# alejandrofontan/AnyFeature-VSLAM

Measured on AMD Instinct MI355X. Metric: keypoints extracted+matched /sec (ORB32, 640x480), higher is better.
Workload: dtype u8; 1 GPU; ORB32 640x480 synthetic corners frames (LCG), 1000 kp/frame budget, 8 levels x1.2, FAST 20; extract+describe on device, brute-force Hamming match frame t vs t-1 (TH 75, ratio 0.6, orientation check); parallelism=frames sharded x1

## Files before the change

### anyfeature-vslam_amd/_lib.py

```python
import ctypes as C
import os

import numpy as np

_HERE = os.path.dirname(os.path.abspath(__file__))
LIB_PATH = os.path.join(_HERE, "libafv_hip.so")


def use_library(path):
    global LIB_PATH
    if _lib is not None:
        raise RuntimeError("the library is already loaded")
    LIB_PATH = os.path.abspath(path)


ABI_VERSION = 6
MAX_LEVELS = 8
DESC_BYTES = 32
OK, EINVAL, ENODEV, ENOMEM, EHIP, ECAPACITY, EUNSUPPORTED, ETIMEOUT = 0, -1, -2, -3, -4, -5, -6, -7
MATCH_KF_KF, MATCH_KF_FRAME = 0, 1
MATCH_FLOAT32 = 0x100
PROJ_LOCALMAP, PROJ_LASTFRAME = 0, 1
STAGES = ("pyramid", "fast_nms", "select_quadtree", "describe", "match_topk", "match_resolve", "retain_harris")

# ... 228 lines not shown
    "afv_points_set_descriptors": (_i, [_vp, _vp, _i, _vp]),
    "afv_points_set_descriptors_from_table": (_i, [_vp, _vp, _i, _vp, _vp, _vp]),
    "afv_points_get": (_i, [_vp, _vp, _i, _vp, _vp, _vp, _vp, _vp, _vp, _vp, _vp, _vp]),
    "afv_frame_set_pose": (_i, [_vp, _vp, _vp, _vp, _f, _f, _f, _f, _f]),
    "afv_frame_search_points": (_i, [_vp, C.POINTER(PointSearch), _vp, _vp, _vp, C.POINTER(C.c_int32)]),
    "afv_frame_fuse_points": (_i, [_vp, C.POINTER(PointSearch), _i, _vp, _vp]),
    "afv_frame_project_points": (_i, [_vp, C.POINTER(PointSearch), C.POINTER(PointProjection)]),
    "afv_frame_pose_optimize": (_i, [_vp, _vp, C.POINTER(PoseJob), _i, C.POINTER(PoseResult)]),
    "afv_table_set_scale": (_i, [_vp, _i, _vp, _vp, _vp, _vp]),
    "afv_table_triangulate": (_i, [_vp, _vp, _vp, C.POINTER(TriPointsJob), _i, _vp, _vp, C.c_int32, _vp, _vp, _vp, _vp, _vp]),
    "afv_table_create_new_points": (_i, [_vp, C.c_int32, _vp, _i, C.POINTER(TableTriJob), C.POINTER(TriPointsJob), _vp, _vp, _vp, C.c_int32,
                                         _vp, _vp, _vp, _vp, _vp, _vp, C.POINTER(C.c_int32)]),
    "afv_table_sim3_hypotheses": (_i, [_vp, _vp, _vp, _vp, C.POINTER(Sim3Job), _i, _vp, _vp, _vp, _vp, _i, _i, _vp, _vp, _vp, _vp, _vp, _vp,
                                       _vp, _vp, _vp]),
    "afv_vocab_set_weights": (_i, [_vp, _vp, _vp, _vp]),
    "afv_bow_vector": (_i, [_vp, _vp, _vp, _i, _vp, _vp, C.POINTER(C.c_int32)]),
    "afv_frame_get_bowvec": (_i, [_vp, _vp, _vp, C.POINTER(C.c_int32)]),
    "afv_table_set_bowvec": (_i, [_vp, _i, _vp, _vp, _i]),
    "afv_table_score_bow": (_i, [_vp, C.POINTER(BowQuery), _i, _vp, _vp, _vp, _vp]),
    "afv_vocab_train": (_i, [_vp, C.POINTER(VocabTrainParams), _vp, C.c_int64, _vp, _i, C.POINTER(_vp)]),
    "afv_vocab_train_device": (_i, [_vp, C.POINTER(VocabTrainParams), _vp, _sz, C.c_int64, _vp, _i, C.POINTER(_vp)]),
    "afv_vocab_tree_nnodes": (_i, [_vp]),
    "afv_vocab_tree_get": (_i, [_vp, _vp, _vp, _vp, _vp, _vp]),
    "afv_vocab_tree_stats": (_i, [_vp, _vp, _vp, _vp, C.POINTER(C.c_int32)]),
    "afv_vocab_tree_destroy": (None, [_vp]),
    "afv_hamming256": (_i, [_vp, _vp]),
    "afv_akaze_default_params": (None, [_vp]),
    "afv_akaze_create": (_i, [_i, _vp, C.POINTER(_vp)]),
    "afv_akaze_destroy": (None, [_vp]),
    "afv_akaze_last_error": (C.c_char_p, [_vp]),
    "afv_akaze_plan_for": (_i, [_vp, _i, _i, _vp]),
    "afv_akaze_scale_space": (_i, [_vp, _vp, _i, _i, _i, _i, C.c_size_t]),
    "afv_akaze_scale_space_device": (_i, [_vp, _vp, _i, _i, _i, _i, C.c_size_t]),
    "afv_akaze_synchronize": (_i, [_vp]),
    "afv_akaze_get_plane": (_i, [_vp, _i, _i, _i, _vp]),
    "afv_akaze_get_kcontrast": (_i, [_vp, _i, _vp]),
    "afv_akaze_detect": (_i, [_vp]),
    "afv_akaze_get_keypoints": (_i, [_vp, _i, _vp, _i, _vp]),
    "afv_akaze_get_candidates": (_i, [_vp, _i, _i, _vp, _i, _vp]),
    "afv_akaze_describe": (_i, [_vp]),
    "afv_akaze_get_features": (_i, [_vp, _i, _vp, _vp, _i, _vp]),
    "afv_akaze_extract": (_i, [_vp, _vp, _i, _i, _i, _i, C.c_size_t, _vp, _vp, _i, _vp]),
    "afv_akaze_extract_device": (_i, [_vp, _vp, _i, _i, _i, _i, C.c_size_t]),
    "afv_akaze_get_quotas": (_i, [_vp, _vp]),
    "afv_akaze_set_step_by_step": (_i, [_vp, _i]),
    "afv_akaze_set_suppress_engine": (_i, [_vp, _i, _i]),
    "afv_akaze_debug_neighbour_cap": (_i, [_vp, _i]),
    "afv_akaze_profile_enable": (_i, [_vp, _i]),
    "afv_akaze_profile_read": (_i, [_vp, _vp, _vp, _vp]),
    "afv_profile_enable": (_i, [_vp, _i]),
    "afv_profile_read": (_i, [_vp, _vp, _vp, _vp]),
    "afv_set_split_threshold": (_i, [_vp, _i]),
    "afv_set_split_chunks": (_i, [_vp, _i]),
    "afv_set_match_engine": (_i, [_vp, _i]),
    "afv_set_small_batch_path": (_i, [_vp, _i, _i]),
    "afv_set_match_resolve": (_i, [_vp, _i]),
    "afv_set_l2_chunk_pairs": (_i, [_vp, _i]),
    "afv_debug_pyramid_plan": (_i, [C.POINTER(OrbParams), _i, _i, _i, _i, _vp, _i, _vp, _vp, _i]),
    "afv_debug_fast_tiles": (_i, [C.POINTER(OrbParams), _i, _i, _vp, _i, _vp, C.POINTER(_i)]),
    "afv_debug_describe_reach": (_i, [_vp, _vp, _vp, _vp, _vp]),
    "afv_set_pipeline_chunk": (_i, [_vp, _i, _i]),
    "afv_get_geometry": (_i, [_vp, C.POINTER(Geometry)]),
    "afv_debug_get_level": (_i, [_vp, _i, _i, _vp]),
    "afv_debug_get_candidates": (_i, [_vp, _i, _i, _vp, _vp, _i, C.POINTER(_i)]),
    "afv_debug_get_selected": (_i, [_vp, _i, _i, _vp, _vp, _vp, _i, C.POINTER(_i)]),
    "afv_debug_blur_level": (_i, [_vp, _i, _i, _vp]),
    "afv_num_stages": (_i, []),
}

_lib = None


def load():
    global _lib
    if _lib is not None:
        return _lib
    try:
        import torch
    except ImportError:
        pass
    if not os.path.exists(LIB_PATH):
        raise ImportError("%s is missing: build the HIP extension first (python __graft_entry__.py or "
                          "anyfeature-vslam_amd/build.py); there is no CPU fallback" % LIB_PATH)
    lib = C.CDLL(LIB_PATH)
    for name, (res, args) in SYMBOLS.items():
        fn = getattr(lib, name)
        fn.restype = res
        fn.argtypes = args
    if lib.afv_abi_version() != ABI_VERSION:
        raise ImportError("%s speaks ABI revision %d, this mirror %d" % (LIB_PATH, lib.afv_abi_version(), ABI_VERSION))
    if lib.afv_num_stages() > len(STAGES):
        raise ImportError("%s reports %d profile stages, this mirror knows %d" % (LIB_PATH, lib.afv_num_stages(), len(STAGES)))
    _lib = lib
    return lib


class AfvError(RuntimeError):
    def __init__(self, code, detail=""):
        self.code = code
        msg = load().afv_strerror(code).decode()
        super().__init__("afv error %d (%s)%s" % (code, msg, (": " + detail) if detail else ""))


def strerror(code):
    return load().afv_strerror(int(code)).decode()

# ... 21 lines not shown
```

### anyfeature-vslam_amd/csrc/afv_api.hip

```cpp
#include "afv_runtime.h"

static const char *k_errors[] = {"ok", "invalid argument", "no usable HIP device", "out of memory", "HIP runtime error",
                                 "output capacity too small", "unsupported", "device-side wait timed out"};


extern "C" void afv_default_orb_params(afv_orb_params *p) {
    if (!p) return;
    p->nfeatures = 1000;
    p->nlevels = 8;
    p->scale_factor = 1.2f;
    p->fast_threshold = 20;
    p->max_width = 640;
    p->max_height = 480;
    p->max_batch = 1;
}

extern "C" int afv_abi_version(void) { return AFV_ABI_VERSION; }

extern "C" const char *afv_strerror(int code) {
    const int i = -code;
    if (i < 0 || i > 7) return "unknown error";
    return k_errors[i];
}
extern "C" const char *afv_last_error(const afv_ctx *ctx) { return ctx ? ctx->last_error.c_str() : ""; }
// ... 124 lines not shown
            float ms = 0.f;
            if (hipEventSynchronize(c->prof_ev[st][i + 1]) == hipSuccess &&
                hipEventElapsedTime(&ms, c->prof_ev[st][i], c->prof_ev[st][i + 1]) == hipSuccess) {
                c->prof_ms[st] += ms;
                c->prof_launches[st] += 1;
            }
        }
        c->prof_used[st] = 0;
    }
}

extern "C" int afv_set_split_threshold(afv_ctx *c, int min_frames) {
    if (!c || min_frames < 2) return AFV_EINVAL;
    c->split_min_frames = min_frames;
    return AFV_OK;
}
extern "C" int afv_set_pipeline_chunk(afv_ctx *c, int frames, int chunks_ahead) {
    if (!c || frames < 1 || chunks_ahead < 1 || chunks_ahead > 64) return AFV_EINVAL;
    c->pipe_chunk = frames;
    c->pipe_ahead = chunks_ahead;
    return AFV_OK;
}
extern "C" int afv_set_match_engine(afv_ctx *c, int engine) {
    if (!c || (engine != AFV_MATCH_ENGINE_POPCOUNT && engine != AFV_MATCH_ENGINE_MFMA)) return AFV_EINVAL;
    c->match_engine = engine;
    return AFV_OK;
}

extern "C" int afv_set_l2_chunk_pairs(afv_ctx *c, int pairs) {
    if (!c || pairs < 1 || pairs > 65535) return AFV_EINVAL;
    c->l2_chunk_pairs = pairs;
    return AFV_OK;
}

extern "C" int afv_set_match_resolve(afv_ctx *c, int engine) {
    if (!c || engine < 0 || engine > 2) return AFV_EINVAL;
    c->resolve_engine = engine;
    return AFV_OK;
}

extern "C" int afv_set_small_batch_path(afv_ctx *c, int mode, int max_frames) {
    if (!c || mode < 0 || mode > 2 || max_frames < 0) return AFV_EINVAL;
    c->small_mode = mode;
    if (max_frames > 0) c->small_max_frames = max_frames;
    return AFV_OK;
}

extern "C" int afv_set_split_chunks(afv_ctx *c, int chunks) {
    if (!c || (chunks != 0 && chunks < 2) || chunks > 64) return AFV_EINVAL;
    c->split_chunks = chunks;
    return AFV_OK;
}

extern "C" int afv_profile_enable(afv_ctx *c, int enable) {
    if (!c) return AFV_EINVAL;
    HIPCHK(c, hipSetDevice(c->device));
    profile_drain(c);
    c->prof = false;
    c->prof_every = enable > 0 ? enable : 0;
    c->prof_tick_extract = c->prof_tick_match = 0;
    if (enable)
        for (int st = 0; st < AFV_NUM_STAGES; ++st) {
            c->prof_ms[st] = 0.f;
            c->prof_launches[st] = 0;
            c->prof_units[st] = 0;
        }
    return AFV_OK;
}

extern "C" int afv_num_stages(void) { return AFV_NUM_STAGES; }

extern "C" int afv_profile_read(afv_ctx *c, int32_t *launches, float *total_ms, int64_t *units) {
    if (!c || !launches || !total_ms) return AFV_EINVAL;
    HIPCHK(c, hipSetDevice(c->device));
    profile_drain(c);
    for (int st = 0; st < AFV_NUM_STAGES; ++st) {
        launches[st] = c->prof_launches[st];
        total_ms[st] = c->prof_ms[st];
        if (units) units[st] = c->prof_units[st];
    }
    return AFV_OK;
}

extern "C" int afv_hamming256(const uint8_t *a, const uint8_t *b) {
    int d = 0;
    for (int i = 0; i < 8; ++i) {
        uint32_t x, y;
        std::memcpy(&x, a + 4 * i, 4);
        std::memcpy(&y, b + 4 * i, 4);
        d += __builtin_popcount(x ^ y);
    }
    return d;
}

static int validate_job(const afv_match_job &j, bool need_angles) {
    if (j.n1 < 0 || j.n2 < 0 || j.n1 > AFV_MAX_SIDE || j.n2 > AFV_MAX_SIDE) return AFV_EINVAL;
    if ((j.n1 > 0 && !j.desc1) || (j.n2 > 0 && !j.desc2)) return AFV_EINVAL;
    if (j.mode & AFV_MATCH_FLOAT32) {
        if (j.desc_bytes < 16 || j.desc_bytes > 4096 || (j.desc_bytes & 15)) return AFV_EINVAL;
    } else if (j.desc_bytes < 1 || j.desc_bytes > 64) {
        return AFV_EINVAL;
    }
    if (j.nnodes1 < 0 || j.nnodes2 < 0) return AFV_EINVAL;
    if (j.nnodes1 > 0 && (!j.node_id1 || !j.seg_ptr1 || !j.seg_idx1)) return AFV_EINVAL;
    if (j.nnodes2 > 0 && (!j.node_id2 || !j.seg_ptr2 || !j.seg_idx2)) return AFV_EINVAL;
    if (need_angles && j.check_orientation && (!j.angle1 || !j.angle2)) return AFV_EINVAL;
// ... 50 lines not shown
}

static int afv_match_triangulation_impl(afv_ctx *c, const afv_tri_job *caller_jobs, int njobs, int32_t *match12, int32_t *nmatches) {
    if (!c || !caller_jobs || njobs < 1 || !match12 || !nmatches) return AFV_EINVAL;
    std::vector<afv_tri_job> loaded;
    if (!afv_load_jobs(caller_jobs, njobs, offsetof(afv_tri_job, u_right1), loaded)) return AFV_EINVAL;
    MatchBatch B;
    B.tri = B.whole_range = true;
    for (int i = 0; i < njobs; ++i) {
        const afv_tri_job &t = loaded[i];
        const int rc = validate_job(t.bow, false);
        if (rc) return rc;
        if ((t.bow.n1 > 0 && (!t.x1 || !t.y1)) || (t.bow.n2 > 0 && (!t.x2 || !t.y2 || !t.sigma2_2))) return AFV_EINVAL;
        if (t.only_stereo != 0 && t.only_stereo != 1) return AFV_EINVAL;
        push_job_sides(B, t.bow, true);
        MatchSide &s1 = B.sides[2 * i], &s2 = B.sides[2 * i + 1];
        s1.x = t.x1, s1.y = t.y1, s1.u_right = t.u_right1;
        s2.x = t.x2, s2.y = t.y2, s2.sigma2 = t.sigma2_2, s2.u_right = t.u_right2;
        B.jobs.push_back(MatchJobSpec{2 * i, 2 * i + 1, t.bow.th_low, t.bow.nnratio, 0, AFV_MATCH_KF_KF, t.F12, t.ex, t.ey, t.only_stereo});
    }
    return afv_match_jobs_run(c, B, match12, nmatches);
}
extern "C" int afv_match_triangulation(afv_ctx *c, const afv_tri_job *jobs, int njobs, int32_t *match12, int32_t *nmatches) {
    return guarded(c, [&] { return afv_match_triangulation_impl(c, jobs, njobs, match12, nmatches); });
}

int afv_check_resolve_guard(afv_ctx *c, const int32_t *nmatches, int n) {
    for (int i = 0; i < n; ++i)
        if (nmatches[i] == AFV_PASS_GUARD) {
            c->last_error = "pair matcher: the fixed point of pair " + std::to_string(i) + " hit its pass guard; afv_set_match_resolve(ctx, 0) selects the ordered walk";
            return AFV_EHIP;
        }
    return AFV_OK;
}

int afv_match_pairs_core(afv_ctx *c, const uint8_t *d_desc, const float *d_ang, int ang_stride, const int32_t *d_n, int cap,
                         const int32_t *d_pair_a, const int32_t *d_pair_b, int npairs, float th_low, float nnratio,
                         int check_orientation, int32_t *d_match, int32_t *d_nmatches, hipStream_t s, int words) {
    c->prof = c->prof_every && (c->prof_tick_match++ % (unsigned)c->prof_every) == 0;
    const int nslices = small_batch_path(c, npairs) ? afv_match_topk_slices(cap, c->match_engine, ((cap + 63) / 64 + 1) / 2) : 1;
    {
        const int rc = ensure_slice_scratch(c, npairs, cap, nslices);
        if (rc) return rc;
    }
    const size_t need = (size_t)npairs * cap * 32;
    if (need > c->topk_bytes) {
        HIPCHK(c, hipDeviceSynchronize());
        if (c->d_topk) (void)hipFree(c->d_topk);
        c->d_topk = nullptr;
        c->topk_bytes = 0;
        HIPCHK(c, hipMalloc(&c->d_topk, need));
        c->topk_bytes = need;
    }
    if (npairs >= c->split_min_frames) {
        HIPCHK(c, hipEventRecord(c->ev_fork, s));
        HIPCHK(c, hipStreamWaitEvent(c->stream2, c->ev_fork, 0));
        const int K = std::max(2, (npairs + 32767) / 32768 * 2);
        for (int k = 0; k < K; ++k) {
            const int b0 = (int)((long)npairs * k / K), e0 = (int)((long)npairs * (k + 1) / K);
            if (e0 <= b0) continue;
            hipStream_t ks = (k & 1) ? c->stream2 : s;
            {
                StageTimer t_(c, AFV_STAGE_MATCH, ks, e0 - b0);
                afv_launch_match_topk(d_desc, d_n, cap, d_pair_a, d_pair_b, e0 - b0, c->d_topk, b0, c->match_engine, nslices, c->d_slice, c->d_tickets, words, ks);
            }
            StageTimer t_(c, AFV_STAGE_MATCH_RESOLVE, ks, e0 - b0);
            afv_launch_match_resolve(d_desc, d_ang, ang_stride, d_n, cap, d_pair_a, d_pair_b, e0 - b0, th_low, nnratio, check_orientation,
                                     d_match, d_nmatches, c->d_topk, b0, resolve_engine_for(c, npairs), words, ks);
        }
        HIPCHK(c, hipEventRecord(c->ev_join, c->stream2));
        HIPCHK(c, hipStreamWaitEvent(s, c->ev_join, 0));
    } else {
        {
            StageTimer t_(c, AFV_STAGE_MATCH, s, npairs);
            afv_launch_match_topk(d_desc, d_n, cap, d_pair_a, d_pair_b, npairs, c->d_topk, 0, c->match_engine, nslices, c->d_slice, c->d_tickets, words, s);
        }
        StageTimer t_(c, AFV_STAGE_MATCH_RESOLVE, s, npairs);
        afv_launch_match_resolve(d_desc, d_ang, ang_stride, d_n, cap, d_pair_a, d_pair_b, npairs, th_low, nnratio, check_orientation, d_match,
                                 d_nmatches, c->d_topk, 0, resolve_engine_for(c, npairs), words, s);
    }
    {
        const hipError_t e = hipGetLastError();
        if (e != hipSuccess) {
            if (nslices > 1 && c->d_tickets) (void)hipMemsetAsync(c->d_tickets, 0, c->tickets_n * sizeof(int), s);
            c->last_error = std::string("pair matcher launch: ") + hipGetErrorString(e);
            return AFV_EHIP;
        }
    }
    return AFV_OK;
}

extern "C" int afv_match_bruteforce_pairs_device(afv_ctx *c, const uint8_t *d_desc, const afv_keypoint *d_kps,
                                                 const int32_t *d_n, int nsets, int cap, const int32_t *d_pair_a,
                                                 const int32_t *d_pair_b, int npairs, float th_low, float nnratio,
                                                 int check_orientation, int32_t *d_match, int32_t *d_nmatches, void *stream) {
    if (!c || !d_desc || !d_n || !d_pair_a || !d_pair_b || !d_match || !d_nmatches) return AFV_EINVAL;
    if (nsets < 1 || npairs < 1 || cap < 1 || cap > 4096) return AFV_EINVAL;
    if (check_orientation && !d_kps) return AFV_EINVAL;
    HIPCHK(c, hipSetDevice(c->device));
    return afv_match_pairs_core(c, d_desc, d_kps ? &d_kps->angle : nullptr, (int)(sizeof(afv_keypoint) / sizeof(float)), d_n, cap,
                                d_pair_a, d_pair_b, npairs, th_low, nnratio, check_orientation, d_match, d_nmatches,
                                stream ? (hipStream_t)stream : c->stream, 8);
}

static int afv_match_l2_impl(afv_ctx *c, const float *desc1, int n1, const float *desc2, int n2, int dim, const uint8_t *valid1,
                            const uint8_t *valid2, float th_low, float nnratio, int32_t *match12, int32_t *nmatches) {
    if (!c || !match12 || !nmatches || n1 < 0 || n2 < 0 || n1 > AFV_MAX_SIDE || n2 > AFV_MAX_SIDE || dim < 1 || dim > 1024)
// ... 363 lines not shown
```

### anyfeature-vslam_amd/csrc/afv_extract.hip

```cpp
#include <chrono>

#include "afv_runtime.h"

int afv_build_geometry(const afv_orb_params &p, int w, int h, int max_batch, Geo &g) {
    std::memset(&g, 0, sizeof(g));
    if (p.nlevels < 1 || p.nlevels > AFV_MAX_LEVELS || w < 1 || h < 1 || w > 4095 || h > 4095) return AFV_EINVAL;
    g.nlevels = p.nlevels;
    g.width = w;
    g.height = h;
    g.fast_threshold = std::min(std::max(p.fast_threshold, 0), 255);
    {
        const float scale = 1.f / ((1 << 2) * 7 * 255.f);
        g.harris_scale4 = scale * scale * scale * scale;
    }
    g.n_ini = (int)roundf((float)w / (float)h);
    if (g.n_ini < 1 || g.n_ini > 16) return AFV_EUNSUPPORTED;
    g.h_x = (float)w / (float)g.n_ini;
    int quota[AFV_MAX_LEVELS], cvq[AFV_MAX_LEVELS];
    afv_level_quotas(p.nfeatures, 1.0f / p.scale_factor, p.nlevels, quota);
    afv_level_quotas(p.nfeatures * 10, (float)(1.0 / (double)p.scale_factor), p.nlevels, cvq);
    size_t pyr_off = 0, cand_off = 0;
    int tile_base = 0, sel_base = 0, desc_blk_base = 0;
    for (int l = 0; l < p.nlevels; ++l) {
        LevelGeo &L = g.lv[l];
// ... 298 lines not shown
        g.lv[l].pyr_off = c->cap_geo.lv[l].pyr_off;
        g.lv[l].pyr_frame_stride = c->cap_geo.lv[l].pyr_frame_stride;
        g.lv[l].cand_off = c->cap_geo.lv[l].cand_off;
        g.lv[l].cand_frame_stride = c->cap_geo.lv[l].cand_frame_stride;
    }
    std::vector<short2> tab(c->tab_elems);
    size_t off = 0;
    for (int l = 1; l < g.nlevels; ++l) {
        c->tab_off_x[l] = off;
        resize_table(g.lv[l - 1].w, g.lv[l].w, tab.data() + off);
        off += (size_t)g.lv[l].w;
        c->tab_off_y[l] = off;
        resize_table(g.lv[l - 1].h, g.lv[l].h, tab.data() + off);
        off += (size_t)g.lv[l].h;
    }
    HIPCHK(c, hipStreamSynchronize(c->stream));
    HIPCHK(c, hipMemcpy(c->d_tab, tab.data(), off * sizeof(short2), hipMemcpyHostToDevice));
    HIPCHK(c, hipMemcpy(c->d_geo, &g, sizeof(Geo), hipMemcpyHostToDevice));
    {
        const int rc_pf = build_pyr_fuse(c, g, tab.data());
        if (rc_pf) return rc_pf;
    }
    c->geo = g;
    c->geo_valid = true;
    return AFV_OK;
}

extern "C" int afv_max_keypoints_per_frame(const afv_ctx *c) {
    if (!c) return AFV_EINVAL;
    int s = 0;
    for (int l = 0; l < c->cap_geo.nlevels; ++l) s += std::max(c->cap_geo.lv[l].quota + 2, 4 * c->cap_geo.n_ini);
    return s;
}

extern "C" int afv_get_geometry(const afv_ctx *c, afv_geometry *g) {
    if (!c || !g) return AFV_EINVAL;
    const Geo &s = c->geo_valid ? c->geo : c->cap_geo;
    std::memset(g, 0, sizeof(*g));
    g->nlevels = s.nlevels;
    g->width = s.width;
    g->height = s.height;
    for (int l = 0; l < s.nlevels; ++l) {
        g->lw[l] = s.lv[l].w;
        g->lh[l] = s.lv[l].h;
        g->lscale[l] = s.lv[l].scale;
        g->quota[l] = s.lv[l].quota;
        g->cv_quota[l] = s.lv[l].cv_quota;
        g->cand_cap[l] = s.lv[l].cand_cap;
    }
    return AFV_OK;
}

static void enqueue_range(afv_ctx *c, const FrameSrc &src, int f0, int nf, afv_keypoint *d_kps, uint8_t *d_desc, int cap, int *d_n,
                          int *d_status, hipStream_t s, bool clear_status = false, const DescribeMirror *mirror = nullptr, bool pyramid_only = false) {
    const Geo &g = c->geo;
    {
        const int per = std::max(std::max(g.total_tiles, afv_describe_blocks_per_frame(&g)), 1);
        const int max_nf = std::max(1, (AFV_MAX_WORK - 8) / per);
        if (nf > max_nf) {
            if (clear_status && d_status) (void)hipMemsetAsync(d_status, 0, sizeof(int), s);
            for (int b = 0; b < nf; b += max_nf) enqueue_range(c, src, f0 + b, std::min(max_nf, nf - b), d_kps, d_desc, cap, d_n, d_status, s, false, mirror, pyramid_only);
            return;
        }
    }
    int *cnt0 = c->d_cand_count + (size_t)f0 * AFV_MAX_LEVELS;
    if (g.nlevels < 2) {
        (void)hipMemsetAsync(cnt0, 0, (size_t)nf * AFV_MAX_LEVELS * sizeof(int), s);
        (void)hipMemsetAsync(c->d_hq_n + f0, 0, sizeof(int), s);
    }
    const bool small = small_batch_path(c, nf);
    if (clear_status && d_status && !(small && c->pf_ok)) (void)hipMemsetAsync(d_status, 0, sizeof(int), s);
    if (small && c->pf_ok) {
        StageTimer t_(c, AFV_STAGE_PYRAMID, s, nf);
        PyrFuseArgs A = c->pf;
        A.zero_counts = cnt0;
        A.n_zero = nf * AFV_MAX_LEVELS;
        A.zero_one = c->d_hq_n + f0;
        A.zero_two = clear_status ? d_status : nullptr;
        afv_launch_pyramid_fused(&src, c->d_pyr, &A, c->pf_lds, f0, nf, s);
    } else {
        StageTimer t_(c, AFV_STAGE_PYRAMID, s, nf);
        for (int l = 1; l < g.nlevels; ++l) {
            const LevelGeo &S = g.lv[l - 1], &D = g.lv[l];
            const uint8_t *sp = (l == 1) ? src.base : c->d_pyr + S.pyr_off;
            const int spitch = (l == 1) ? src.stride : S.pitch;
            const size_t sframe = (l == 1) ? src.frame_stride : S.pyr_frame_stride;
            afv_launch_resize(sp, S.w, S.h, spitch, sframe, c->d_pyr + D.pyr_off, D.w, D.h, D.pitch, D.pyr_frame_stride,
                              c->d_tab + c->tab_off_x[l], c->d_tab + c->tab_off_y[l], f0, nf, l == 1 ? cnt0 : nullptr, nf * AFV_MAX_LEVELS,
                              l == 1 ? c->d_hq_n + f0 : nullptr, s);
        }
    }
    if (pyramid_only) return;
    {
        StageTimer t_(c, AFV_STAGE_FAST_NMS, s, nf);
        afv_launch_fast_nms(c->d_geo, g.total_tiles, &src, c->d_pyr, c->d_cand_packed, c->d_cand_count, f0, nf, s);
    }
    {
        StageTimer t_(c, AFV_STAGE_HARRIS, s, nf);
        afv_launch_retain_harris(c->d_geo, g.nlevels, &src, c->d_pyr, c->d_cand_packed, c->d_cand_count, c->d_l1, c->d_l1_count,
                                 c->d_l1_resp, c->d_hq + (size_t)f0 * c->hq_per_frame, c->d_hq_n + f0, f0, nf, small ? 1 : 0, s);
    }
    {
        StageTimer t_(c, AFV_STAGE_SELECT, s, nf);
        afv_launch_select(c->d_geo, g.nlevels, c->d_l1, c->d_l1_resp, c->d_l1_count, c->d_kept_xy, c->d_kept_resp,
                          c->d_kept_node, c->d_sel, c->d_sel_count, c->select_M, f0, nf, (small && c->select_wide_ok) ? 1 : 0, s);
    }
    {
        StageTimer t_(c, AFV_STAGE_DESCRIBE, s, nf);
        afv_launch_describe(c->d_geo, afv_describe_blocks_per_frame(&g), &src, c->d_pyr, c->d_sel, c->d_sel_count, d_kps, d_desc, cap, d_n,
                            d_status, f0, nf, mirror, s);
    }
}

static int enqueue_extract(afv_ctx *c, const FrameSrc &src, int nframes, afv_keypoint *d_kps, uint8_t *d_desc, int cap,
                           int *d_n, int *d_status, hipStream_t s) {
    if (nframes >= c->split_min_frames) {
        if (d_status) HIPCHK(c, hipMemsetAsync(d_status, 0, sizeof(int), s));
        HIPCHK(c, hipEventRecord(c->ev_fork, s));
        HIPCHK(c, hipStreamWaitEvent(c->stream2, c->ev_fork, 0));
        const int K = c->split_chunks ? c->split_chunks : std::min(64, 2 * std::max(1, (int)((float)nframes / 170.0f + 0.45f)));
        for (int k = 0; k < K; ++k) {
            const int b = (int)((long)nframes * k / K), e = (int)((long)nframes * (k + 1) / K);
            if (e > b) enqueue_range(c, src, b, e - b, d_kps, d_desc, cap, d_n, d_status, (k & 1) ? c->stream2 : s);
        }
        HIPCHK(c, hipEventRecord(c->ev_join, c->stream2));
        HIPCHK(c, hipStreamWaitEvent(s, c->ev_join, 0));
    } else {
        enqueue_range(c, src, 0, nframes, d_kps, d_desc, cap, d_n, d_status, s, true);
    }
    HIPCHK(c, hipGetLastError());
    c->last_src = src;
    c->last_nframes = nframes;
    return AFV_OK;
}

static int begin_call(afv_ctx *c, int width, int height, bool timed = true) {
    HIPCHK(c, hipSetDevice(c->device));
    const int rc = set_geometry(c, width, height);
    if (rc) return rc;
    c->prof = timed && c->prof_every && (c->prof_tick_extract++ % (unsigned)c->prof_every) == 0;
    return AFV_OK;
}

static FrameSrc staged_src(const afv_ctx *c, int width, int height) {
    const size_t pitch = align_up((size_t)width, 64);
    return FrameSrc{c->d_frames, (int)pitch, align_up(pitch * (size_t)height, 256)};
}

static int stage_images(afv_ctx *c, const uint8_t *const *frames, int f0, int nf, int width, int height, int stride_bytes, bool pinned,
                        size_t gather_off, bool join, hipStream_t s) {
    const FrameSrc src = staged_src(c, width, height);
    const size_t pitch = (size_t)src.stride, fstride = src.frame_stride, frame_bytes = (size_t)width * height;
    uint8_t *gathered = c->h_stage + gather_off;
    if (!pinned) {
        for (int f = f0; f < f0 + nf; ++f) {
            uint8_t *dst = gathered + (size_t)f * frame_bytes;
            if ((size_t)stride_bytes == (size_t)width) {
                std::memcpy(dst, frames[f], frame_bytes);
            } else {
                for (int y = 0; y < height; ++y) std::memcpy(dst + (size_t)y * width, frames[f] + (size_t)y * stride_bytes, (size_t)width);
            }
        }
    }
    bool linear = pitch == (size_t)width && (join ? fstride == frame_bytes : nf == 1);
    if (pinned) {
        linear = linear && join && (size_t)stride_bytes == (size_t)width;
        for (int f = f0 + 1; f < f0 + nf && linear; ++f) linear = frames[f] == frames[f - 1] + frame_bytes;
    }
    if (linear) {
        HIPCHK(c, hipMemcpyAsync(c->d_frames + (size_t)f0 * fstride, pinned ? frames[f0] : gathered + (size_t)f0 * frame_bytes, frame_bytes * (size_t)nf,
                                 hipMemcpyHostToDevice, s));
        return AFV_OK;
    }
    for (int f = f0; f < f0 + nf; ++f) {
        const uint8_t *sp = pinned ? frames[f] : gathered + (size_t)f * frame_bytes;
        HIPCHK(c, hipMemcpy2DAsync(c->d_frames + (size_t)f * fstride, pitch, sp, pinned ? (size_t)stride_bytes : (size_t)width, (size_t)width,
// ... 420 lines not shown
```

### anyfeature-vslam_amd/csrc/afv_runtime.h

```cpp
#pragma once
#include <cstdio>
#include <cstdlib>
#include <cstring>
#include <unordered_map>
#include <vector>

#include "afv_device.h"
#include "afv_host.h"
#include "afv_jobs.h"

extern "C" void afv_launch_resize(const uint8_t *src, int sw, int sh, int spitch, size_t sframe, uint8_t *dst, int dw, int dh,
                                  int dpitch, size_t dframe, const short2 *xt, const short2 *yt, int frame_base, int nframes, int *zero_counts,
                                  int n_zero, int *zero_one, hipStream_t stream);
extern "C" int afv_resize_window_ok(int sw, int sh, int dw, int dh);
extern "C" void afv_launch_pyramid_fused(const FrameSrc *src0, uint8_t *pyr, const PyrFuseArgs *args, size_t lds_bytes, int frame_base, int nframes,
                                         hipStream_t stream);
extern "C" int afv_pyramid_fused_prepare(size_t lds_bytes);
extern "C" void afv_launch_fast_nms(const Geo *geo, int total_tiles, const FrameSrc *src0, const uint8_t *pyr, uint32_t *cand_packed,
                                    int *cand_count, int frame_base, int nframes, hipStream_t stream);
extern "C" size_t afv_harris_queue_per_frame(const Geo *g);
extern "C" void afv_launch_retain_harris(const Geo *geo_dev, int nlevels, const FrameSrc *src0, const uint8_t *pyr,
                                         const uint32_t *cand_packed, const int *cand_count, uint32_t *l1, int *l1_count,
                                         float *l1_resp, uint2 *queue, int *queue_n, int frame_base, int nframes, int small, hipStream_t stream);
extern "C" size_t afv_select_lds_bytes(int M);
// ... 256 lines not shown
    int *d_bow_n = nullptr;
    bool has_bow = false;
    int bow_n = 0;
    float *d_depth = nullptr;
    int *d_sad = nullptr, *d_best_r = nullptr, *d_nstereo = nullptr;
    bool has_depth = false;
    bool has_stereo = false;
    uint8_t *d_pyr = nullptr;
    size_t pyr_bytes = 0, pyr_off[AFV_MAX_LEVELS]{};
    int pyr_levels = 0, pyr_w[AFV_MAX_LEVELS]{}, pyr_h[AFV_MAX_LEVELS]{};
    bool has_pyramid = false;
    bool has_pose = false;
    float Rcw[9]{}, tcw[3]{}, Ow[3]{}, fx = 0, fy = 0, cx = 0, cy = 0, mbf = 0;
};

struct afv_points {
    afv_ctx *c = nullptr;
    int cap = 0;
    int desc_bytes = 32, words = 8, float_dim = 0;
    uint8_t *d_block = nullptr;
    DevPointPlanes P{};
    uint8_t *d_stage = nullptr;
    size_t stage_bytes = 0;
    uint8_t *h_pin = nullptr;
    size_t pin_bytes = 0;
    hipEvent_t ev = nullptr;
    bool ev_armed = false;
};

#define AFV_MAX_SIDE 8192

struct afv_ctx {
    int device = 0;
    hipStream_t stream = nullptr;
    hipStream_t stream2 = nullptr;
    hipEvent_t ev_fork = nullptr, ev_join = nullptr;
    hipStream_t stream_copy = nullptr;
    std::vector<hipEvent_t> pipe_ev;
    int pipe_chunk = 64;
    int pipe_ahead = 8;
    int split_min_frames = 64;
    int match_engine = AFV_MATCH_ENGINE_MFMA;
    int resolve_engine = 2;
    int resolve_wg_max_pairs = 256;
    int proj_engine = 2;
    int proj_wg_lds_max = 0;
    int frame_lds_max = 0;
    int *d_proj_ticket = nullptr;
    int *d_points_count = nullptr;
    int proj_fuse = 1;
    std::vector<afv_frame *> frames;
    std::vector<afv_points *> points;
    int split_chunks = 0;
    int small_mode = 1;
    int small_max_frames = 4;
    int pf_tw = 16, pf_th = 8;
    bool pf_ok = false;
    PyrFuseArgs pf{};
    size_t pf_lds = 0;
    uint8_t *d_pf_blob = nullptr;
    size_t pf_blob_cap = 0;
    afv_orb_params p{};
    Geo geo{};
    Geo cap_geo{};
    Geo *d_geo = nullptr;
    bool geo_valid = false;
    short2 *d_tab = nullptr;
    size_t tab_off_x[AFV_MAX_LEVELS]{}, tab_off_y[AFV_MAX_LEVELS]{};
    size_t tab_elems = 0;
    uint8_t *d_pyr = nullptr;
    uint32_t *d_cand_packed = nullptr, *d_kept_xy = nullptr;
    uint32_t *d_l1 = nullptr;
    float *d_l1_resp = nullptr;
    int *d_l1_count = nullptr;
    uint2 *d_hq = nullptr;
    int *d_hq_n = nullptr;
    size_t hq_per_frame = 0;
    float *d_kept_resp = nullptr;
    uint16_t *d_kept_node = nullptr;
    int *d_cand_count = nullptr, *d_sel_count = nullptr;
    SelPoint *d_sel = nullptr;
    int select_M = 64;
    bool select_wide_ok = true;
    uint8_t *d_frames = nullptr;
    size_t frames_pitch = 0, frames_stride = 0;
    uint8_t *d_out_block = nullptr;
    size_t out_kps_off = 0, out_desc_off = 0, out_bytes = 0;
    afv_keypoint *d_kps = nullptr;
    uint8_t *d_desc = nullptr;
    int *d_n = nullptr, *d_status = nullptr;
    int stage_cap = 0;
    uint8_t *d_match = nullptr;
    size_t match_bytes = 0;
    uint8_t *h_stage = nullptr;
    size_t stage_bytes = 0;
    bool stage_pinned = false;
    void *d_topk = nullptr;
    size_t topk_bytes = 0;
    void *d_l2_scratch = nullptr;
    size_t l2_bytes = 0;
    int l2_chunk_pairs = 2048;
    void *d_slice = nullptr;
    size_t slice_bytes = 0;
    int *d_tickets = nullptr;
    size_t tickets_n = 0;
    FrameSrc last_src{};
// ... 327 lines not shown
```

### anyfeature-vslam_amd/extractor.py

```python
import ctypes as C
import enum

import numpy as np

from . import _lib
from ._lib import KP_DTYPE, AfvError, ptr


class CovarianceMethod(enum.IntEnum):
    SIZE = 1
    NONE = 0


class FeatureExtractorSettings:
    numOctaves0 = 8
    scaleFactor0 = 1.2
    th0 = 20.0

    def __init__(self, settings=None):
        if settings is not None and settings != "none":
            if isinstance(settings, str):
                import yaml
                with open(settings) as fh:
                    text = fh.read()
# ... 125 lines not shown
        if kps is None:
            kps = torch.empty((B, cap, 7), dtype=torch.float32, device=dev)
        if desc is None:
            desc = torch.empty((B, cap, 32), dtype=torch.uint8, device=dev)
        if n_out is None:
            n_out = torch.empty((B,), dtype=torch.int32, device=dev)
        if status is None:
            status = torch.empty((1,), dtype=torch.int32, device=dev)
        rc = _lib.launch_ordered(self, dev, stream, lambda s: self.lib.afv_orb_extract_batch_device(
            self.handle, frames.data_ptr(), B, W, H, frames.stride(1), frames.stride(0), kps.data_ptr(), desc.data_ptr(), cap,
            n_out.data_ptr(), status.data_ptr(), s), (frames, kps, desc, n_out, status))
        self.check(rc, "afv_orb_extract_batch_device")
        return kps, desc, n_out, status

    def size_sigma(self, kps):
        kps = np.ascontiguousarray(kps, KP_DTYPE)
        n = len(kps)
        size = np.zeros(n, np.float32); s2 = np.zeros(n, np.float32); inf = np.zeros(n, np.float32)
        self.check(self.lib.afv_orb_size_sigma(self.handle, ptr(kps), n, ptr(size), ptr(s2), ptr(inf)))
        return size, s2, inf

    def profile_enable(self, enable=True, every=1):
        self.check(self.lib.afv_profile_enable(self.handle, int(every) if enable else 0))

    def profile_read(self):
        ns = max(int(self.lib.afv_num_stages()), len(_lib.STAGES))
        launches = np.zeros(ns, np.int32); ms = np.zeros(ns, np.float32)
        units = np.zeros(ns, np.int64)
        self.check(self.lib.afv_profile_read(self.handle, ptr(launches), ptr(ms), ptr(units)))
        return {name: {"launches": int(launches[i]), "total_ms": float(ms[i]), "units": int(units[i])}
                for i, name in enumerate(_lib.STAGES)}

    def set_split_threshold(self, min_frames):
        self.check(self.lib.afv_set_split_threshold(self.handle, int(min_frames)))

    def set_pipeline_chunk(self, frames, chunks_ahead=8):
        self.check(self.lib.afv_set_pipeline_chunk(self.handle, int(frames), int(chunks_ahead)))

    def set_match_engine(self, engine):
        self.check(self.lib.afv_set_match_engine(self.handle, int(engine)))

    def set_small_batch_path(self, mode, max_frames=0):
        self.check(self.lib.afv_set_small_batch_path(self.handle, int(mode), int(max_frames)))

    def set_l2_chunk_pairs(self, pairs):
        self.check(self.lib.afv_set_l2_chunk_pairs(self.handle, int(pairs)))

    def set_match_resolve(self, engine):
        self.check(self.lib.afv_set_match_resolve(self.handle, int(engine)))

    def set_split_chunks(self, chunks):
        self.check(self.lib.afv_set_split_chunks(self.handle, int(chunks)))

    @property
    def stream(self):
        return self.lib.afv_stream(self.handle)

    def debug_level(self, frame, level):
        g = self.geometry()
        out = np.zeros((g["lh"][level], g["lw"][level]), np.uint8)
        self.check(self.lib.afv_debug_get_level(self.handle, frame, level, ptr(out)))
        return out

    def debug_blur_level(self, frame, level):
        g = self.geometry()
        out = np.zeros((g["lh"][level], g["lw"][level]), np.uint8)
        self.check(self.lib.afv_debug_blur_level(self.handle, frame, level, ptr(out)))
        return out

    def debug_candidates(self, frame, level):
        g = self.geometry()
        cap = g["cand_cap"][level]
        packed = np.zeros(cap, np.uint32); resp = np.zeros(cap, np.float32)
        n = C.c_int(0)
        self.check(self.lib.afv_debug_get_candidates(self.handle, frame, level, ptr(packed), ptr(resp), cap, C.byref(n)))
        packed = packed[:n.value]
        return (packed & 4095).astype(np.int32), ((packed >> 12) & 4095).astype(np.int32), (packed >> 24).astype(np.int32), \
            resp[:n.value].copy()

    def debug_selected(self, frame, level):
        g = self.geometry()
        cap = g["quota"][level] + 8
        x = np.zeros(cap, np.int32); y = np.zeros(cap, np.int32); r = np.zeros(cap, np.float32)
        n = C.c_int(0)
        self.check(self.lib.afv_debug_get_selected(self.handle, frame, level, ptr(x), ptr(y), ptr(r), cap, C.byref(n)))
        return x[:n.value].copy(), y[:n.value].copy(), r[:n.value].copy()


class FeatureExtractor_orb32:

    def __init__(self, nfeatures, settings=None, device=0, max_width=640, max_height=480, max_batch=1):
        self.settings = settings or FeatureExtractorSettings()
        self.nfeatures = int(nfeatures)
        s = self.settings
        self.ctx = Context(self.nfeatures, s.nOctaves, s.scaleFactor, int(s.detectTh), max_width, max_height, max_batch, device)
        self.mvScaleFactor = [1.0]
        for _ in range(1, s.nOctaves):
            self.mvScaleFactor.append(float(np.float32(self.mvScaleFactor[-1]) * np.float32(s.scaleFactor)))
        self.mnFeaturesPerLevel = self.ctx.geometry()["quota"]

    def GetLevels(self):
        return self.settings.nOctaves

    def GetScaleFactor(self):
        return self.settings.scaleFactor

# ... 46 lines not shown
```

### include/afv_hip.h

```cpp
#ifndef AFV_HIP_H
#define AFV_HIP_H
#include <stddef.h>
#include <stdint.h>
#ifdef __cplusplus
extern "C" {
#endif

#define AFV_MAX_LEVELS 8
#define AFV_DESC_BYTES 32

enum {
    AFV_OK = 0,
    AFV_EINVAL = -1,
    AFV_ENODEV = -2,
    AFV_ENOMEM = -3,
    AFV_EHIP = -4,
    AFV_ECAPACITY = -5,
    AFV_EUNSUPPORTED = -6,
    AFV_ETIMEOUT = -7
};

#define AFV_ABI_VERSION 6
int afv_abi_version(void);

// ... 332 lines not shown
int afv_vocab_set_weights(afv_ctx *ctx, afv_vocab *v, const double *weight, const int32_t *word_id);
int afv_bow_vector(afv_ctx *ctx, const afv_vocab *v, const int32_t *leaf_node, int n, int32_t *word, double *value, int32_t *n_out);
int afv_frame_get_bowvec(afv_frame *f, int32_t *word, double *value, int32_t *n_out);
int afv_table_set_bowvec(afv_table *t, int slot, const int32_t *word, const double *value, int n);

#define AFV_BOW_QUERY_SLOT 0
#define AFV_BOW_QUERY_FRAME 1
#define AFV_BOW_QUERY_HOST 2
typedef struct afv_bow_query {
    uint32_t struct_size;
    int32_t kind;
    int32_t slot;
    int32_t n;
    afv_frame *frame;
    const int32_t *word;
    const double *value;
} afv_bow_query;
int afv_table_score_bow(afv_table *t, const afv_bow_query *q, int nq, const uint8_t *slot_mask, int32_t *common, double *score,
                        int32_t *first_common);

#define AFV_VOCAB_TRAIN_MAX_ROWS (1 << 26)
typedef struct afv_vocab_train_params {
    uint32_t struct_size;
    int32_t k;
    int32_t L;
    int32_t desc_bytes;
    uint64_t seed;
    int32_t max_iters;
    int32_t n_init;
    const uint8_t *init_centres;
} afv_vocab_train_params;
typedef struct afv_vocab_tree afv_vocab_tree;
int afv_vocab_train(afv_ctx *ctx, const afv_vocab_train_params *params, const uint8_t *desc, int64_t n, const int32_t *image_ptr, int nimages,
                    afv_vocab_tree **out);
int afv_vocab_train_device(afv_ctx *ctx, const afv_vocab_train_params *params, const uint8_t *d_desc, size_t pitch_bytes, int64_t n,
                           const int32_t *image_ptr, int nimages, afv_vocab_tree **out);
int afv_vocab_tree_nnodes(const afv_vocab_tree *t);
int afv_vocab_tree_get(const afv_vocab_tree *t, int32_t *parent, uint8_t *desc, uint8_t *is_leaf, double *weight, int32_t *ni);
int afv_vocab_tree_stats(const afv_vocab_tree *t, int32_t *rounds, int64_t *rows, double *seconds, int32_t *capped);
void afv_vocab_tree_destroy(afv_vocab_tree *t);

int afv_hamming256(const uint8_t *a, const uint8_t *b);

enum { AFV_STAGE_PYRAMID = 0, AFV_STAGE_FAST_NMS = 1 , AFV_STAGE_SELECT = 2, AFV_STAGE_DESCRIBE = 3,
       AFV_STAGE_MATCH = 4 , AFV_STAGE_MATCH_RESOLVE = 5 ,
       AFV_STAGE_HARRIS = 6 ,
       AFV_NUM_STAGES = 7 };
int afv_num_stages(void);
int afv_profile_enable(afv_ctx *ctx, int enable);
int afv_profile_read(afv_ctx *ctx, int32_t *launches , float *total_ms ,
                     int64_t *units );
int afv_set_split_threshold(afv_ctx *ctx, int min_frames);
int afv_set_split_chunks(afv_ctx *ctx, int chunks);
int afv_set_l2_chunk_pairs(afv_ctx *ctx, int pairs);
int afv_set_match_resolve(afv_ctx *ctx, int engine);
int afv_set_small_batch_path(afv_ctx *ctx, int mode, int max_frames);
enum { AFV_MATCH_ENGINE_POPCOUNT = 0, AFV_MATCH_ENGINE_MFMA = 1 };
int afv_set_match_engine(afv_ctx *ctx, int engine);
int afv_set_pipeline_chunk(afv_ctx *ctx, int frames, int chunks_ahead);

typedef struct {
    int32_t nlevels, width, height;
    int32_t lw[AFV_MAX_LEVELS], lh[AFV_MAX_LEVELS];
    float lscale[AFV_MAX_LEVELS];
    int32_t quota[AFV_MAX_LEVELS];
    int32_t cv_quota[AFV_MAX_LEVELS];
    int32_t cand_cap[AFV_MAX_LEVELS];
} afv_geometry;
int afv_get_geometry(const afv_ctx *ctx, afv_geometry *g);
int afv_debug_get_level(afv_ctx *ctx, int frame, int level, uint8_t *out);
int afv_debug_get_candidates(afv_ctx *ctx, int frame, int level, uint32_t *packed, float *response, int cap, int *n_out);
int afv_debug_get_selected(afv_ctx *ctx, int frame, int level, int32_t *x, int32_t *y, float *response, int cap, int *n_out);
int afv_debug_blur_level(afv_ctx *ctx, int frame, int level, uint8_t *out);
int afv_debug_pyramid_plan(const afv_orb_params *params, int width, int height, int tile_w, int tile_h, int16_t *regions,
                           int regions_cap, int32_t *info, int16_t *tables, int tables_cap);

int afv_debug_fast_tiles(const afv_orb_params *params, int width, int height, int32_t *tiles, int tiles_cap, int32_t *level_wh, int *n_out);

int afv_debug_describe_reach(uint8_t *R, uint16_t *items, uint16_t *dwords, int32_t *counts, int32_t *layout);

#ifdef __cplusplus
}
#endif
#endif
```

Measured before the change: 221.4 million keypoints/s.

## Add split schedule: pyramid halves first, then interleaved chunks across two streams

```diff
diff --git a/anyfeature-vslam_amd/_lib.py b/anyfeature-vslam_amd/_lib.py
--- a/anyfeature-vslam_amd/_lib.py
+++ b/anyfeature-vslam_amd/_lib.py
@@ -304,6 +304,7 @@
     "afv_profile_read": (_i, [_vp, _vp, _vp, _vp]),
     "afv_set_split_threshold": (_i, [_vp, _i]),
     "afv_set_split_chunks": (_i, [_vp, _i]),
+    "afv_set_split_schedule": (_i, [_vp, _i]),
     "afv_set_match_engine": (_i, [_vp, _i]),
     "afv_set_small_batch_path": (_i, [_vp, _i, _i]),
     "afv_set_match_resolve": (_i, [_vp, _i]),
diff --git a/anyfeature-vslam_amd/csrc/afv_api.hip b/anyfeature-vslam_amd/csrc/afv_api.hip
--- a/anyfeature-vslam_amd/csrc/afv_api.hip
+++ b/anyfeature-vslam_amd/csrc/afv_api.hip
@@ -200,6 +200,12 @@
     return AFV_OK;
 }
 
+extern "C" int afv_set_split_schedule(afv_ctx *c, int mode) {
+    if (!c || (mode != 0 && mode != 1)) return AFV_EINVAL;
+    c->split_schedule = mode;
+    return AFV_OK;
+}
+
 extern "C" int afv_profile_enable(afv_ctx *c, int enable) {
     if (!c) return AFV_EINVAL;
     HIPCHK(c, hipSetDevice(c->device));
@@ -356,7 +362,8 @@
         HIPCHK(c, hipMalloc(&c->d_topk, need));
         c->topk_bytes = need;
     }
-    if (npairs >= c->split_min_frames) {
+    const bool split = npairs >= c->split_min_frames && (c->split_schedule == 0 || npairs > 4096);
+    if (split) {
         HIPCHK(c, hipEventRecord(c->ev_fork, s));
         HIPCHK(c, hipStreamWaitEvent(c->stream2, c->ev_fork, 0));
         const int K = std::max(2, (npairs + 32767) / 32768 * 2);
diff --git a/anyfeature-vslam_amd/csrc/afv_extract.hip b/anyfeature-vslam_amd/csrc/afv_extract.hip
--- a/anyfeature-vslam_amd/csrc/afv_extract.hip
+++ b/anyfeature-vslam_amd/csrc/afv_extract.hip
@@ -374,25 +374,28 @@
 }
 
 static void enqueue_range(afv_ctx *c, const FrameSrc &src, int f0, int nf, afv_keypoint *d_kps, uint8_t *d_desc, int cap, int *d_n,
-                          int *d_status, hipStream_t s, bool clear_status = false, const DescribeMirror *mirror = nullptr, bool pyramid_only = false) {
+                          int *d_status, hipStream_t s, bool clear_status = false, const DescribeMirror *mirror = nullptr, bool pyramid_only = false,
+                          bool pyramid_done = false) {
     const Geo &g = c->geo;
     {
         const int per = std::max(std::max(g.total_tiles, afv_describe_blocks_per_frame(&g)), 1);
         const int max_nf = std::max(1, (AFV_MAX_WORK - 8) / per);
         if (nf > max_nf) {
             if (clear_status && d_status) (void)hipMemsetAsync(d_status, 0, sizeof(int), s);
-            for (int b = 0; b < nf; b += max_nf) enqueue_range(c, src, f0 + b, std::min(max_nf, nf - b), d_kps, d_desc, cap, d_n, d_status, s, false, mirror, pyramid_only);
+            for (int b = 0; b < nf; b += max_nf)
+                enqueue_range(c, src, f0 + b, std::min(max_nf, nf - b), d_kps, d_desc, cap, d_n, d_status, s, false, mirror, pyramid_only, pyramid_done);
             return;
         }
     }
     int *cnt0 = c->d_cand_count + (size_t)f0 * AFV_MAX_LEVELS;
-    if (g.nlevels < 2) {
+    if (g.nlevels < 2 && !pyramid_done) {
         (void)hipMemsetAsync(cnt0, 0, (size_t)nf * AFV_MAX_LEVELS * sizeof(int), s);
         (void)hipMemsetAsync(c->d_hq_n + f0, 0, sizeof(int), s);
     }
     const bool small = small_batch_path(c, nf);
     if (clear_status && d_status && !(small && c->pf_ok)) (void)hipMemsetAsync(d_status, 0, sizeof(int), s);
-    if (small && c->pf_ok) {
+    if (pyramid_done) {
+    } else if (small && c->pf_ok) {
         StageTimer t_(c, AFV_STAGE_PYRAMID, s, nf);
         PyrFuseArgs A = c->pf;
         A.zero_counts = cnt0;
@@ -441,9 +444,29 @@
         HIPCHK(c, hipEventRecord(c->ev_fork, s));
         HIPCHK(c, hipStreamWaitEvent(c->stream2, c->ev_fork, 0));
         const int K = c->split_chunks ? c->split_chunks : std::min(64, 2 * std::max(1, (int)((float)nframes / 170.0f + 0.45f)));
-        for (int k = 0; k < K; ++k) {
-            const int b = (int)((long)nframes * k / K), e = (int)((long)nframes * (k + 1) / K);
-            if (e > b) enqueue_range(c, src, b, e - b, d_kps, d_desc, cap, d_n, d_status, (k & 1) ? c->stream2 : s);
+        if (c->split_schedule == 0) {
+            for (int k = 0; k < K; ++k) {
+                const int b = (int)((long)nframes * k / K), e = (int)((long)nframes * (k + 1) / K);
+                if (e > b) enqueue_range(c, src, b, e - b, d_kps, d_desc, cap, d_n, d_status, (k & 1) ? c->stream2 : s);
+            }
+        } else {
+            const int Ks = (K + 1) / 2, K2 = K / 2;
+            const double px = std::max(1.0, (double)c->geo.width * (double)c->geo.height);
+            const int lead = std::min(nframes / 10, std::max(1, (int)(28.0 * 640.0 * 480.0 / px + 0.5)));
+            const int h = std::min(nframes, (int)(((long)nframes * Ks + K - 1) / K) + (lead + 1) / 2);
+            enqueue_range(c, src, 0, h, d_kps, d_desc, cap, d_n, d_status, s, false, nullptr, true);
+            HIPCHK(c, hipMemsetAsync(c->d_hq_n, 0, (size_t)h * sizeof(int), s));
+            if (nframes > h) {
+                enqueue_range(c, src, h, nframes - h, d_kps, d_desc, cap, d_n, d_status, c->stream2, false, nullptr, true);
+                HIPCHK(c, hipMemsetAsync(c->d_hq_n + h, 0, (size_t)(nframes - h) * sizeof(int), c->stream2));
+            }
+            for (int k = 0; k < Ks; ++k) {
+                const int b = (int)((long)h * k / Ks), e = (int)((long)h * (k + 1) / Ks);
+                if (e > b) enqueue_range(c, src, b, e - b, d_kps, d_desc, cap, d_n, d_status, s, false, nullptr, false, true);
+                if (k >= K2) continue;
+                const int b2 = h + (int)((long)(nframes - h) * k / K2), e2 = h + (int)((long)(nframes - h) * (k + 1) / K2);
+                if (e2 > b2) enqueue_range(c, src, b2, e2 - b2, d_kps, d_desc, cap, d_n, d_status, c->stream2, false, nullptr, false, true);
+            }
         }
         HIPCHK(c, hipEventRecord(c->ev_join, c->stream2));
         HIPCHK(c, hipStreamWaitEvent(s, c->ev_join, 0));
diff --git a/anyfeature-vslam_amd/csrc/afv_runtime.h b/anyfeature-vslam_amd/csrc/afv_runtime.h
--- a/anyfeature-vslam_amd/csrc/afv_runtime.h
+++ b/anyfeature-vslam_amd/csrc/afv_runtime.h
@@ -332,6 +332,7 @@
     std::vector<afv_frame *> frames;
     std::vector<afv_points *> points;
     int split_chunks = 0;
+    int split_schedule = 1;
     int small_mode = 1;
     int small_max_frames = 4;
     int pf_tw = 16, pf_th = 8;
diff --git a/anyfeature-vslam_amd/extractor.py b/anyfeature-vslam_amd/extractor.py
--- a/anyfeature-vslam_amd/extractor.py
+++ b/anyfeature-vslam_amd/extractor.py
@@ -201,6 +201,9 @@
     def set_split_chunks(self, chunks):
         self.check(self.lib.afv_set_split_chunks(self.handle, int(chunks)))
 
+    def set_split_schedule(self, mode):
+        self.check(self.lib.afv_set_split_schedule(self.handle, int(mode)))
+
     @property
     def stream(self):
         return self.lib.afv_stream(self.handle)
diff --git a/include/afv_hip.h b/include/afv_hip.h
--- a/include/afv_hip.h
+++ b/include/afv_hip.h
@@ -408,6 +408,7 @@
                      int64_t *units );
 int afv_set_split_threshold(afv_ctx *ctx, int min_frames);
 int afv_set_split_chunks(afv_ctx *ctx, int chunks);
+int afv_set_split_schedule(afv_ctx *ctx, int mode);
 int afv_set_l2_chunk_pairs(afv_ctx *ctx, int pairs);
 int afv_set_match_resolve(afv_ctx *ctx, int engine);
 int afv_set_small_batch_path(afv_ctx *ctx, int mode, int max_frames);
```

After: 225.3 million keypoints/s (median of 6 runs). 1.7% higher.
